# gfxdisp/FovVideoVDP

Hardware: AMD Instinct MI355X
Metric: Mpixels/s (test+ref) at 4Kx60f; JOD delta vs reference (higher is better)
Workload: dtype f32

## Files before the change

fovvideovdp_amd/csrc/aux_kernels.hpp:

```cpp
#pragma once
struct FinalizeArgs {
    const float* partial;
    float* Q;
    int n_bands, n, q_stride, q_col0, tc;
    float inv_beta;
    int nblk[FVVDP_MAX_BANDS];
    long long off[FVVDP_MAX_BANDS];
    float npx[FVVDP_MAX_BANDS];
};

__device__ __forceinline__ void finalize_one(const FinalizeArgs& a, const int b, const int cc, const int s, const int lane) {
    float q = 0.0f;
    if (cc < a.tc) {
        const float* p = a.partial + a.off[b] + (size_t)s * a.nblk[b] * 2 + cc;
        double sum = 0.0;
        for (int k = lane; k < a.nblk[b]; k += 64) sum += (double)p[2 * k];
#pragma unroll
        for (int off = 32; off > 0; off >>= 1) sum += __shfl_down(sum, off, 64);
        q = (float)pow(sum / (double)a.npx[b], (double)a.inv_beta);
    }
    if (lane == 0) a.Q[((size_t)b * 2 + cc) * a.q_stride + a.q_col0 + s] = q;
}

__global__ __launch_bounds__(64) void finalize_kernel(const FinalizeArgs a) {
    const int i = blockIdx.x;
    finalize_one(a, i / (2 * a.n), (i / a.n) % 2, i % a.n, (int)threadIdx.x);
}

struct PoolArgs {
    const float* Q;
    int n_bands, n_ch, n_frames, q_stride;
    float beta_sch, beta_tch, beta_t, w_transient, jod_a, beta_jod;
    float* out;
};

__device__ __forceinline__ float pool_pow(float x, float p) { return p == 1.0f ? x : powf(x, p); }

__device__ __forceinline__ float pool_frame(const PoolArgs& a, const int f) {
    float qt = 0.0f;
    for (int c = 0; c < a.n_ch; ++c) {
        const float wc = (a.n_ch == 2 && c == 1) ? a.w_transient : 1.0f;
        float qs = 0.0f;
        for (int b = 0; b < a.n_bands; ++b)
            qs += pool_pow(fabsf(a.Q[((size_t)b * 2 + c) * a.q_stride + f] * wc), a.beta_sch);
        qs = pool_pow(qs, 1.0f / a.beta_sch);
        qt += pool_pow(qs, a.beta_tch);
    }
    qt = pool_pow(qt, 1.0f / a.beta_tch);
    return pool_pow(qt, a.beta_t);
}

__device__ __forceinline__ void pool_jod_body(const PoolArgs& a, double* s_part, const int tid) {
    double acc = 0.0;
    if (tid < 256) {
        for (int f = tid; f < a.n_frames; f += 256) acc += (double)pool_frame(a, f);
        s_part[tid] = acc;
    }
    __syncthreads();
    for (int o = 128; o >= 1; o >>= 1) {
        if (tid < o) s_part[tid] += s_part[tid + o];
        __syncthreads();
    }
    if (tid == 0) {
        const float q_all = pool_pow((float)(s_part[0] / (double)a.n_frames), 1.0f / a.beta_t);
        const float sgn = a.jod_a < 0.0f ? -1.0f : 1.0f;
        a.out[0] = sgn * powf(powf(fabsf(a.jod_a), 1.0f / a.beta_jod) * q_all, a.beta_jod) + 10.0f;
    }
}

__global__ __launch_bounds__(256) void pool_jod_kernel(const PoolArgs a) {
    __shared__ double s_part[256];
    pool_jod_body(a, s_part, (int)threadIdx.x);
}

struct PoolColsArgs {
    PoolArgs p;
    int n_cols;
};
// ... 209 lines not shown
```

fovvideovdp_amd/csrc/fvvdp_hip.hip:

```cpp
#include <hip/hip_runtime.h>
#include <hip/hip_fp16.h>

#include <algorithm>
#include <cmath>
#include <cfloat>
#include <cstdarg>
#include <cstdio>
#include <cstdlib>
#include <cstring>
#include <vector>

#include "fvvdp_hip.h"
#include "fvvdp_hip_images.h"
#include "fvvdp_hip_gaze.h"

static thread_local char g_err[512] = "";

static int fail(int code, const char* fmt, ...) {
    va_list ap;
    va_start(ap, fmt);
    vsnprintf(g_err, sizeof(g_err), fmt, ap);
    va_end(ap);
    return code;
}
// ... 37 lines not shown
};
static CtxEnv read_env() {
    CtxEnv e;
    auto num = [](const char* name, int dflt) { const char* v = getenv(name); return (v && v[0]) ? atoi(v) : dflt; };
    if (const char* v = getenv("FVVDP_ALLOC")) e.alloc_malloc = strcmp(v, "malloc") == 0;
    e.vmm_chunk = (size_t)(num("FVVDP_VMM_CHUNK_MB", 0) > 0 ? num("FVVDP_VMM_CHUNK_MB", 0) : 0) << 20;
    e.probe_n = num("FVVDP_PLACEMENT_PROBE", -1);
    e.probe_extra = num("FVVDP_PLACEMENT_EXTRA", -1);
    if (const char* v = getenv("FVVDP_PLACEMENT_MIXED_TBS")) e.probe_mixed = (float)atof(v);
    if (const char* v = getenv("FVVDP_BAND_INRANGE")) e.inrange_off = v[0] == '0';
    if (const char* v = getenv("FVVDP_BAND_FUSE")) e.fuse_mode = (v[0] == '0' || v[0] == '1') ? v[0] - '0' : -1;
    e.band2_kr = num("FVVDP_BAND2_KR", 0);
    e.band2_kr2 = num("FVVDP_BAND2_KR2", -1);
    e.band2_wpb = num("FVVDP_BAND2_WPB", 0);
    if (const char* v = getenv("FVVDP_K1_TICKET")) e.k1_ticket = v[0] != '0' ? 1 : 0;
    if (const char* v = getenv("FVVDP_BAND2_TICKET")) e.band2_ticket = v[0] != '0' ? 1 : 0;
    if (const char* v = getenv("FVVDP_LEVEL0_SPLIT")) e.level0_split = v[0] != '0' ? 1 : 0;
    e.temporal_scalar = getenv("FVVDP_TEMPORAL_SCALAR") != nullptr;
    e.debug_variant = getenv("FVVDP_DEBUG_VARIANT") != nullptr;
    e.yuv_general = getenv("FVVDP_YUV_GENERAL_MATRIX") != nullptr;
    e.gaze_group = num("FVVDP_GAZE_GROUP", 0);
    return e;
}

struct VmmBlock {
    void* ptr;
    size_t size;
    std::vector<hipMemGenericAllocationHandle_t> handles;
};
struct fvvdp_ctx {
    CtxEnv env;
    int W = 0, H = 0, n_bands = 0, P = 0, max_frames = 0;
    fvvdp_params prm{};
    double rho_band[FVVDP_MAX_BANDS + 1]{};
    int lw[FVVDP_MAX_BANDS + 1]{}, lh[FVVDP_MAX_BANDS + 1]{};
    float* level[FVVDP_MAX_BANDS + 1]{};
    float* level0_hi = nullptr;
    int sel_phase = 9;
    int sel_n = 0;
    int sel_kept = -1;
    float sel_us[8] = {0, 0, 0, 0, 0, 0, 0, 0};
    int level0_kind = 0;
    int level0_kind_hi = -1;
    long long n_sync = 0, n_alloc = 0, n_free = 0;
    bool created = false;
    bool lum_known = false;
    int lum_state = 0;
    int lum_hold = 0;
    int lum_top = 0;
    float lum_lo = 0.0f, lum_hi = 0.0f, lum_width = 0.0f;
    float* partial = nullptr;
    long long partial_off[FVVDP_MAX_BANDS]{};
    int max_blk[FVVDP_MAX_BANDS]{};
    int* d_ticket = nullptr;
    size_t partial_floats = 0;
    float4* csf = nullptr;
    float4* csf_y = nullptr;
    bool csf_set = false;
    float y_first = 0, y_inv_step = 0, y_lo = 0, y_hi = 0;
    std::vector<float> h_lut3[2];
    float h_axes[3][FVVDP_LUT_N]{};
    float* d_axes = nullptr;
    float4* sublut[FVVDP_MAX_BANDS]{};
    float4* rmap[FVVDP_MAX_BANDS]{};
    int sub_rw[FVVDP_MAX_BANDS]{}, sub_ilo[FVVDP_MAX_BANDS]{};
    fvvdp_geom sub_geom{};
    const float* map_vx[FVVDP_MAX_BANDS]{};
    const float* map_vy[FVVDP_MAX_BANDS]{};
    const float* map_rm[FVVDP_MAX_BANDS]{};
    float map_rm_max[FVVDP_MAX_BANDS]{}, map_rm_min[FVVDP_MAX_BANDS]{};
    bool maps_set = false;
    bool sub_valid = false;
    float rho_lo = 0, rho_hi = 0, ecc_lo = 0, ecc_hi = 0;
    bool lut3_set[2] = {false, false};
    float* d_fix = nullptr;
    float* d_taps = nullptr;
    int* d_idx = nullptr;
    float* lum_buf = nullptr;
    size_t lum_floats = 0;
    float* heat[FVVDP_MAX_BANDS + 1]{};
    unsigned int* colour_ws = nullptr;
    size_t scratch = 0;
    std::vector<VmmBlock> vmm;
    long long wave_capacity = 4096;
    long long wave_capacity2 = 4096;
    bool timing = false;
    std::vector<std::pair<hipEvent_t, hipEvent_t>> ev[FVVDP_MAX_BANDS + 2];
    float t_ms[FVVDP_MAX_BANDS + 2]{};
    int t_cnt[FVVDP_MAX_BANDS + 2]{};
};

static const size_t VMM_MIN_BYTES = (size_t)16 << 20;
static const size_t VMM_BIG_BYTES = (size_t)256 << 20;

static int vmm_alloc(fvvdp_ctx* c, void** out, size_t bytes);
static void vmm_free_all(fvvdp_ctx* c);

template <typename T>
static int dev_alloc(fvvdp_ctx* c, T** p, size_t count) {
    void* q = nullptr;
    const size_t bytes = count * sizeof(T);
    if (!c->env.alloc_malloc && bytes >= VMM_MIN_BYTES && vmm_alloc(c, &q, bytes) == FVVDP_OK) {
    } else {
        q = nullptr;
        (void)hipGetLastError();
        hipError_t e = hipMalloc(&q, bytes);
        if (e != hipSuccess) return fail(FVVDP_ENOMEM, "hipMalloc(%zu bytes) failed: %s", bytes, hipGetErrorString(e));
// ... 147 lines not shown

static void choose_level0(fvvdp_ctx* c);

extern "C" int fvvdp_ctx_create(fvvdp_ctx** out, int width, int height, int n_bands, int planes, int max_frames,
                                const double* h_rho_band, const fvvdp_params* prm) {
    if (!out || !prm || !h_rho_band) return fail(FVVDP_EINVAL, "null argument");
    if (planes != 2 && planes != 4) return fail(FVVDP_EINVAL, "planes must be 2 (image) or 4 (video), got %d", planes);
    if (n_bands < 1 || n_bands > FVVDP_MAX_BANDS) return fail(FVVDP_EINVAL, "n_bands %d out of range", n_bands);
    if (max_frames < 1) return fail(FVVDP_EINVAL, "max_frames must be >= 1");
    if (width < 4 || height < 4) return fail(FVVDP_EINVAL, "frame %dx%d too small", width, height);
    fvvdp_ctx* c = new fvvdp_ctx();
    c->env = read_env();
    c->W = width;
    c->H = height;
    c->n_bands = n_bands;
    c->P = planes;
    c->max_frames = max_frames;
    c->prm = *prm;
    int w = width, h = height;
    for (int i = 0; i <= n_bands; ++i) {
        c->lw[i] = w;
        c->lh[i] = h;
        c->rho_band[i] = h_rho_band[i];
        if (i < n_bands && (w < 2 || h < 2)) {
            delete c;
            return fail(FVVDP_EINVAL, "pyramid level %d is %dx%d: too many bands for this frame size", i, w, h);
        }
        w = (w + 1) / 2;
        h = (h + 1) / 2;
    }
    int rc = FVVDP_OK;
    for (int i = 0; i <= n_bands && rc == FVVDP_OK; ++i) {
        rc = dev_alloc(c, &c->level[i], (size_t)max_frames * c->lw[i] * c->lh[i] * planes);
    }
    size_t off = 0;
    for (int b = 0; b < n_bands; ++b) {
        const int n_strips = band_strips(c->lw[b + 1]);
        const int max_chunks = (c->lh[b + 1] + 1) / 2;
        c->max_blk[b] = n_strips * max_chunks;
    }
    for (int b = 0; b + 1 < n_bands; ++b) {
        const int blk2 = band2_strips(c->lw[b + 1]) * c->lh[b + 2];
        if (blk2 > c->max_blk[b]) c->max_blk[b] = blk2;
        if (blk2 > c->max_blk[b + 1]) c->max_blk[b + 1] = blk2;
    }
    for (int b = 0; b < n_bands; ++b) {
        c->partial_off[b] = (long long)off;
        off += (size_t)max_frames * c->max_blk[b] * 2;
    }
    c->partial_floats = off;
    if (rc == FVVDP_OK) rc = dev_alloc(c, &c->partial, off);
    if (rc == FVVDP_OK) {
        float* q = nullptr;
        rc = dev_alloc(c, &q, 16);
        c->d_ticket = reinterpret_cast<int*>(q);
    }
    if (rc == FVVDP_OK) rc = dev_alloc(c, &c->csf, (size_t)n_bands * FVVDP_LUT_N);
    if (rc == FVVDP_OK) rc = dev_alloc(c, &c->csf_y, (size_t)FVVDP_LUT_N);
    if (rc == FVVDP_OK) rc = dev_alloc(c, &c->d_fix, (size_t)max_frames * 2);
    if (rc == FVVDP_OK) rc = dev_alloc(c, &c->d_taps, (size_t)2 * FVVDP_MAX_TAPS);
    if (rc == FVVDP_OK) rc = dev_alloc(c, &c->d_idx, (size_t)max_frames + FVVDP_MAX_TAPS);
    if (rc != FVVDP_OK) {
        fvvdp_ctx_destroy(c);
        return rc;
    }
    {
        int dev = 0, cus = 256, per_cu = 16;
        if (hipGetDevice(&dev) == hipSuccess) {
            hipDeviceProp_t prop;
            if (hipGetDeviceProperties(&prop, dev) == hipSuccess) cus = prop.multiProcessorCount;
        }
        hipError_t e = (planes == 4)
            ? hipOccupancyMaxActiveBlocksPerMultiprocessor(&per_cu, band_kernel<4, false, 0>, 64, 0)
            : hipOccupancyMaxActiveBlocksPerMultiprocessor(&per_cu, band_kernel<2, false, 0>, 64, 0);
        if (e != hipSuccess || per_cu < 1) per_cu = 16;
        c->wave_capacity = (long long)per_cu * cus;
        int per_cu2 = 16;
        e = (planes == 4) ? hipOccupancyMaxActiveBlocksPerMultiprocessor(&per_cu2, band2_kernel<4, false>, 64, 0)
                          : hipOccupancyMaxActiveBlocksPerMultiprocessor(&per_cu2, band2_kernel<2, false>, 64, 0);
        if (e != hipSuccess || per_cu2 < 1) per_cu2 = 16;
        c->wave_capacity2 = (long long)per_cu2 * cus;
    }
    choose_level0(c);
    if (!c->level[0]) {
        fvvdp_ctx_destroy(c);
        return fail(FVVDP_ENOMEM, "no device memory for pyramid level 0");
    }
    c->created = true;
    *out = c;
    return FVVDP_OK;
}

extern "C" void fvvdp_ctx_destroy(fvvdp_ctx* c) {
    if (!c) return;
    (void)hipDeviceSynchronize();
    for (int i = 0; i <= FVVDP_MAX_BANDS; ++i)
        dev_free(c, c->level[i]);
    dev_free(c, c->level0_hi);
    dev_free(c, c->partial);
    dev_free(c, c->d_ticket);
    if (c->csf) (void)hipFree(c->csf);
    if (c->csf_y) (void)hipFree(c->csf_y);
    for (int i = 0; i <= FVVDP_MAX_BANDS; ++i)
        dev_free(c, c->heat[i]);
    if (c->colour_ws) (void)hipFree(c->colour_ws);
    if (c->d_fix) (void)hipFree(c->d_fix);
    if (c->d_taps) (void)hipFree(c->d_taps);
    if (c->d_idx) (void)hipFree(c->d_idx);
// ... 167 lines not shown
    return lo >= c->prm.lbkg_min &&
           c->prm.contrast_max * lo > c->lum_width &&
           lo >= 2.0f * c->y_lo && hi <= 0.5f * c->y_hi;
}

static int temporal_channels_core(fvvdp_ctx* c, const void* d_test, const void* d_ref, int dtype, int C,
                                  size_t chan_stride, size_t frame_stride, const fvvdp_eotf* eotf,
                                  const float* h_rgb2y, const int32_t* h_frame_idx, const int32_t* h_frame_idx1,
                                  const float* h_taps, int fl, int n_out, int slot0, int32_t* d_oob_flag, void* stream) {
    if (!c || !d_test || !d_ref || !eotf || !h_frame_idx || !h_taps) return fail(FVVDP_EINVAL, "null argument");
    if (dtype < FVVDP_U8 || dtype > FVVDP_F32) return fail(FVVDP_EINVAL, "Only uint8, uint16 and float32 is currently supported");
    if (C != 1 && C != 3) return fail(FVVDP_EINVAL, "The content must have either 1 or 3 colour channels.");
    if (C == 3 && !h_rgb2y) return fail(FVVDP_EINVAL, "rgb2y weights required for C == 3");
    if (fl < 1 || fl > FVVDP_MAX_TAPS) return fail(FVVDP_EINVAL, "filter length %d out of range", fl);
    if (c->P == 2 && fl != 1) return fail(FVVDP_EINVAL, "still-image context (planes == 2) needs fl == 1");
    if (n_out < 1 || slot0 < 0 || slot0 + n_out > c->max_frames) return fail(FVVDP_EINVAL, "slots [%d,%d) exceed max_frames %d", slot0, slot0 + n_out, c->max_frames);
    if (eotf->kind == FVVDP_EOTF_LUT && (dtype == FVVDP_F32 || !eotf->d_lut)) return fail(FVVDP_EINVAL, "FVVDP_EOTF_LUT needs an integer source and a table");
    if (eotf->kind != FVVDP_EOTF_LUT && dtype == FVVDP_U8) return fail(FVVDP_EINVAL, "uint8 sources need FVVDP_EOTF_LUT (uint16: table or closed form)");
    hipStream_t st = reinterpret_cast<hipStream_t>(stream);
    const int HW = c->W * c->H;
    luminance_slots(c, slot0, n_out);
    luminance_range(c, eotf, C, h_rgb2y, h_taps, fl);
    Timed tm(c, 0, st);
    const bool ring64 = (c->P == 4) && fl > 32 && fl <= 64 && !c->env.temporal_scalar &&
                        k1_ring64_ok(dtype, C, eotf->kind);
    const bool ring_ok = ((c->P == 4) && (fl <= 32)) || ring64;
    if (ring_ok) {
        const int FL = fl <= 8 ? 8 : (fl <= 16 ? 16 : (fl <= 32 ? 32 : 64));
        const int max_out = T_MAX_IDX - (FL - 1);
        auto run = [&](int t_begin, int t_end) -> int {
            for (int t0 = t_begin; t0 < t_end; t0 += max_out) {
                const int nn = (t_end - t0) < max_out ? (t_end - t0) : max_out;
                TemporalArgs a;
                memset(&a, 0, sizeof(a));
                a.src[0] = d_test;
                a.src[1] = d_ref;
                a.chan_stride = chan_stride;
                a.frame_stride = frame_stride;
                a.C = C;
                a.HW = HW;
                a.e = make_eotf(eotf);
                if (C == 3) { a.w[0] = h_rgb2y[0]; a.w[1] = h_rgb2y[1]; a.w[2] = h_rgb2y[2]; } else { a.w[0] = 1.0f; }
                a.n_out = nn;
                a.fl = fl;
                a.out = level_addr(c, 0, slot0 + t0);
                a.oob = d_oob_flag;
                for (int k = 0; k < fl; ++k) { a.taps2[k][0] = h_taps[k]; a.taps2[k][1] = h_taps[fl + k]; }
                const int pad = FL - fl;
                for (int u = 0; u < FL - 1 + nn; ++u) {
                    const int src = t0 + u - pad;
                    a.idx[u] = h_frame_idx[src < 0 ? 0 : src];
                    a.idx1[u] = h_frame_idx1 ? h_frame_idx1[src < 0 ? 0 : src] : a.idx[u];
                }
                const int PXv = k1_px(FL);
                const int es = dtype == FVVDP_U8 ? 1 : (dtype == FVVDP_U16 ? 2 : 4);
                const bool vec_ok = !c->env.temporal_scalar && (HW % PXv == 0) && (HW >= PXv) &&
                                    (chan_stride % PXv == 0) && (frame_stride % PXv == 0) &&
                                    (reinterpret_cast<uintptr_t>(d_test) % (size_t)(es * PXv) == 0) &&
                                    (reinterpret_cast<uintptr_t>(d_ref) % (size_t)(es * PXv) == 0);
                if (vec_ok) {
                    const bool tickets = FL == 16 && c->env.k1_ticket != 0;
                    if (tickets && dtype == FVVDP_U8 && c->d_ticket) {
                        if (hipMemsetAsync(c->d_ticket, 0, sizeof(int), st) == hipSuccess) a.ticket = c->d_ticket;
                        else (void)hipGetLastError();
                    }
                    k1_launch_vec(FL, dtype, a, st);
                } else if (FL == 64) {
                    return fail(FVVDP_EINVAL, "source pointers must be aligned to their element size");
                } else {
                    k1_launch_ring(FL, dtype, a, st);
                }
            }
            return FVVDP_OK;
        };
        {
            const int rc = run(0, n_out);
            if (rc != FVVDP_OK) return rc;
        }
    } else if (c->P == 4 && fl > 32 && fl <= 64 && !h_frame_idx1 && !c->env.temporal_scalar &&
               fl - 1 + n_out <= T_MAX_IDX && k1_ring64_ok(FVVDP_F32, 1, FVVDP_EOTF_NONE)) {
        const int total = fl - 1 + n_out;
        std::vector<int> uniq(h_frame_idx, h_frame_idx + total);
        std::sort(uniq.begin(), uniq.end());
        uniq.erase(std::unique(uniq.begin(), uniq.end()), uniq.end());
        const int nu = (int)uniq.size();
        {
            const int rc = grow_lum_buf(c, (size_t)2 * nu * HW, fl, st);
            if (rc != FVVDP_OK) return rc;
        }
        LumArgs la;
        memset(&la, 0, sizeof(la));
        la.src[0] = d_test;
        la.src[1] = d_ref;
        la.chan_stride = chan_stride;
        la.frame_stride = frame_stride;
        la.C = C;
        la.HW = HW;
        la.e = make_eotf(eotf);
        if (C == 3) { la.w[0] = h_rgb2y[0]; la.w[1] = h_rgb2y[1]; la.w[2] = h_rgb2y[2]; } else { la.w[0] = 1.0f; }
        la.n_frames = nu;
        la.out = c->lum_buf;
        la.oob = d_oob_flag;
        for (int k = 0; k < nu; ++k) la.fr[k] = uniq[k];
        k1_launch_luminance(dtype, la, st);
        std::vector<int32_t> pos(total);
        for (int u = 0; u < total; ++u) pos[u] = (int32_t)(std::lower_bound(uniq.begin(), uniq.end(), h_frame_idx[u]) - uniq.begin());
        fvvdp_eotf none;
        memset(&none, 0, sizeof(none));
        none.kind = FVVDP_EOTF_NONE;
        HIP_TRY(hipGetLastError());
        const bool timing = c->timing;
        c->timing = false;
        c->lum_hold += 1;
        const int rc2 = temporal_channels_core(c, c->lum_buf, c->lum_buf + (size_t)nu * HW, FVVDP_F32, 1, 0, (size_t)HW, &none, nullptr,
                                               pos.data(), nullptr, h_taps, fl, n_out, slot0, d_oob_flag, stream);
        c->timing = timing;
        c->lum_hold -= 1;
        return rc2;
    } else {
        if (h_frame_idx1) return fail(FVVDP_EINVAL, "per-frame source pointers are supported for video with fl <= 32 (uint8: 64) only");
        if (fl - 1 + n_out > c->max_frames + FVVDP_MAX_TAPS) return fail(FVVDP_EINVAL, "too many frames for one call");
        GenericArgs a;
        memset(&a, 0, sizeof(a));
        if (fl <= 32 && fl - 1 + n_out <= T_MAX_IDX) {
            a.inline_tables = 1;
            for (int k = 0; k < 2 * fl; ++k) a.taps_i[k] = h_taps[k];
            for (int k = 0; k < fl - 1 + n_out; ++k) a.idx_i[k] = h_frame_idx[k];
        } else {
            HIP_TRY(hipStreamSynchronize(st));
            c->n_sync += 1;
            HIP_TRY(hipMemcpy(c->d_taps, h_taps, sizeof(float) * 2 * fl, hipMemcpyHostToDevice));
            HIP_TRY(hipMemcpy(c->d_idx, h_frame_idx, sizeof(int) * (fl - 1 + n_out), hipMemcpyHostToDevice));
        }
        a.src[0] = d_test;
        a.src[1] = d_ref;
        a.chan_stride = chan_stride;
        a.frame_stride = frame_stride;
        a.C = C;
        a.HW = HW;
        a.e = make_eotf(eotf);
        if (C == 3) { a.w[0] = h_rgb2y[0]; a.w[1] = h_rgb2y[1]; a.w[2] = h_rgb2y[2]; } else { a.w[0] = 1.0f; }
        a.n_out = n_out;
        a.fl = fl;
        a.out = level_addr(c, 0, slot0);
        a.oob = d_oob_flag;
        a.taps = c->d_taps;
        a.idx = c->d_idx;
        k1_launch_generic(c->P, dtype, a, st);
    }
    HIP_TRY(hipGetLastError());
    return FVVDP_OK;
}

extern "C" int fvvdp_temporal_channels(fvvdp_ctx* c, const void* d_test, const void* d_ref, int dtype, int C,
                                       size_t chan_stride, size_t frame_stride, const fvvdp_eotf* eotf,
                                       const float* h_rgb2y, const int32_t* h_frame_idx, const float* h_taps, int fl,
                                       int n_out, int slot0, int32_t* d_oob_flag, void* stream) {
    return temporal_channels_core(c, d_test, d_ref, dtype, C, chan_stride, frame_stride, eotf, h_rgb2y, h_frame_idx, nullptr,
                                  h_taps, fl, n_out, slot0, d_oob_flag, stream);
}

extern "C" int fvvdp_temporal_channels_frames(fvvdp_ctx* c, const void* const* h_test_frames, const void* const* h_ref_frames,
                                              int n_frames, int dtype, int C, size_t chan_stride, const fvvdp_eotf* eotf,
                                              const float* h_rgb2y, const int32_t* h_frame_idx, const float* h_taps, int fl,
                                              int n_out, int slot0, int32_t* d_oob_flag, void* stream) {
    if (!c || !h_test_frames || !h_ref_frames || !h_frame_idx) return fail(FVVDP_EINVAL, "null argument");
    if (n_frames < 1 || n_frames > 65536) return fail(FVVDP_EINVAL, "n_frames out of range");
    if (dtype < FVVDP_U8 || dtype > FVVDP_F32) return fail(FVVDP_EINVAL, "Only uint8, uint16 and float32 is currently supported");
    if (fl < 1 || fl > ((eotf && k1_ring64_ok(dtype, C, eotf->kind)) ? 64 : 32) || c->P != 4)
        return fail(FVVDP_EUNSUPPORTED, "per-frame source pointers: video contexts with fl <= 32 (uint8, float luminance: 64) only");
    const size_t es = dtype == FVVDP_U8 ? 1 : (dtype == FVVDP_U16 ? 2 : 4);
    const void* const* fr[2] = {h_test_frames, h_ref_frames};
    uintptr_t base[2];
    size_t gran = 4;
    for (int s = 0; s < 2; ++s) {
        base[s] = UINTPTR_MAX;
        for (int i = 0; i < n_frames; ++i) {
            if (!fr[s][i]) return fail(FVVDP_EINVAL, "null frame pointer");
            const uintptr_t p = reinterpret_cast<uintptr_t>(fr[s][i]);
            if (p % es) return fail(FVVDP_EINVAL, "frame pointer not aligned to its element size");
            if (p < base[s]) base[s] = p;
        }
        for (int i = 0; i < n_frames; ++i)
            if ((reinterpret_cast<uintptr_t>(fr[s][i]) - base[s]) % (es * 4)) gran = 1;
    }
    std::vector<int32_t> off[2];
    for (int s = 0; s < 2; ++s) {
        off[s].resize(n_frames);
        for (int i = 0; i < n_frames; ++i) {
            const uintptr_t d = (reinterpret_cast<uintptr_t>(fr[s][i]) - base[s]) / (es * gran);
            if (d > 0x7FFFFFFFu) return fail(FVVDP_EUNSUPPORTED, "frames are too far apart in memory for 31-bit frame indices");
            off[s][i] = (int32_t)d;
        }
    }
    const int total = fl - 1 + n_out;
    std::vector<int32_t> i0(total), i1(total);
    for (int u = 0; u < total; ++u) {
        const int f = h_frame_idx[u];
        if (f < 0 || f >= n_frames) return fail(FVVDP_EINVAL, "frame index %d out of range", f);
        i0[u] = off[0][f];
        i1[u] = off[1][f];
    }
    return temporal_channels_core(c, reinterpret_cast<const void*>(base[0]), reinterpret_cast<const void*>(base[1]), dtype, C,
// ... 408 lines not shown
            a.mrm = c->map_rm[b];
        }
        a.rho_band = (float)c->rho_band[b];
        a.rho_lo = c->rho_lo;
        a.rho_hi = c->rho_hi;
        a.ecc_lo = c->ecc_lo;
        a.ecc_hi = c->ecc_hi;
        for (int ax = 0; ax < 3; ++ax) {
            a.first[ax] = c->h_axes[ax][0];
            a.inv_step[ax] = (float)(FVVDP_LUT_N - 1) / (c->h_axes[ax][FVVDP_LUT_N - 1] - c->h_axes[ax][0]);
            const double step = ((double)c->h_axes[ax][FVVDP_LUT_N - 1] - (double)c->h_axes[ax][0]) / (FVVDP_LUT_N - 1);
            a.frac_scale[ax] = (float)(step / (step + 1e-6));
            a.grid_off[ax] = -a.first[ax] * a.inv_step[ax];
        }
        a.frame_w = c->W;
        a.frame_h = c->H;
        a.rmap = geom ? c->rmap[b] : nullptr;
        a.rmap_w = (c->lw[b] + 1) / 2;
    }
    {
        const size_t lut_b = (size_t)FOV_PLANE * c->sub_rw[b] * sizeof(float4);
        const size_t lds_static = sizeof(float4) * FVVDP_LUT_N + sizeof(float2) * 3 * FVVDP_LUT_N;
        a.lut_lds = (fov && lut_b <= 56 * 1024 && lut_b + (size_t)c->lh[b] * sizeof(float) + lds_static <= 64 * 1024) ? 1 : 0;
    }
}

static int bands_forward_core(fvvdp_ctx* c, int slot0, int n, float* d_Q, int q_stride, int q_col0, const float* h_fixation,
                              const fvvdp_geom* geom, const fvvdp_band_maps* maps, const fvvdp_pool_params* pool,
                              float* d_jod, void* stream, int plan_n = 0) {
    if (plan_n < 1) plan_n = n;
    if (!c || !d_Q) return fail(FVVDP_EINVAL, "null argument");
    if (slot0 < 0 || n < 1 || slot0 + n > c->max_frames) return fail(FVVDP_EINVAL, "slots [%d,%d) exceed max_frames %d", slot0, slot0 + n, c->max_frames);
    if (pool) {
        if (!d_jod) return fail(FVVDP_EINVAL, "null argument");
        int rc = check_pool_params(pool);
        if (rc != FVVDP_OK) return rc;
    }
    const bool last_batch = (q_col0 + n == q_stride);
    const bool pool_now = pool && last_batch;
    if (n < 1 || n > c->max_frames) return fail(FVVDP_EINVAL, "n=%d exceeds max_frames=%d", n, c->max_frames);
    if (q_col0 < 0 || q_col0 + n > q_stride) return fail(FVVDP_EINVAL, "Q columns out of range");
    const bool fov = h_fixation != nullptr;
    if (fov && !geom && !c->maps_set) return fail(FVVDP_EINVAL, "foveated mode needs the display geometry (or fvvdp_ctx_set_view_maps)");
    if (fov && !(c->lut3_set[0] && (c->P == 2 || c->lut3_set[1]))) return fail(FVVDP_ESTATE, "fvvdp_ctx_set_csf_3d not called");
    if (!fov && !c->csf_set) return fail(FVVDP_ESTATE, "fvvdp_ctx_set_csf_1d not called");
    hipStream_t st = reinterpret_cast<hipStream_t>(stream);
    if (fov) {
        HIP_TRY(hipMemcpyAsync(c->d_fix, h_fixation, sizeof(float) * 2 * n, hipMemcpyHostToDevice, st));
        int rc = build_sublut(c, geom, st);
        if (rc != FVVDP_OK) return rc;
    }
    FinalizeArgs fa;
    memset(&fa, 0, sizeof(fa));
    bool any_maps = false;
    if (maps)
        for (int b = 0; b < c->n_bands; ++b) any_maps = any_maps || maps[b].d_D || maps[b].d_contrast || maps[b].d_lbkg || maps[b].d_S;
    const int fuse_mode = c->env.fuse_mode;
    const bool fuse_ok = !fov && !any_maps && fuse_mode != 0;
    for (int b = 0; b < c->n_bands; ++b) {
        const bool big = (long long)c->lw[b] * c->lh[b] >= 500000;
        if (fuse_ok && (big || fuse_mode == 1) && b + 1 < c->n_bands && c->lw[b + 1] >= 4 && c->lh[b + 1] >= 4 &&
            c->lw[b + 2] >= 2 && c->lh[b + 2] >= 2) {
            Band2Args a;
            memset(&a, 0, sizeof(a));
            a.A = level_addr(c, b, b == 0 ? slot0 : 0);
            a.Gc = c->level[b + 2];
            a.w = c->lw[b];
            a.h = c->lh[b];
            a.wb = c->lw[b + 1];
            a.hb = c->lh[b + 1];
            a.wc = c->lw[b + 2];
            a.hc = c->lh[b + 2];
            a.n_strips = band2_strips(a.wb);
            chunking2(a.hc, a.n_strips, plan_n, c->wave_capacity2, c->env.band2_kr, a.n_chunks, a.kr);
            a.n_big = a.n_chunks;
            a.kr2 = a.kr;
            a.n_frames = n;
            {
                const long long waves = (long long)plan_n * a.n_strips * a.n_chunks;
                int kr2 = (waves >= 2 * c->wave_capacity2 && a.n_chunks >= 3 && a.kr >= 16) ? (a.kr + 3) / 4 : 0;
                if (c->env.band2_kr2 >= 0) kr2 = c->env.band2_kr2;
                if (kr2 >= 1 && kr2 < a.kr && a.n_chunks >= 2) {
                    a.n_big = a.n_chunks - 1;
                    a.kr2 = kr2;
                    a.n_chunks = a.n_big + (a.hc - a.n_big * a.kr + kr2 - 1) / kr2;
                }
            }
            a.mulA = (b == 0) ? 1.0f : 2.0f;
            a.mulB = 2.0f;
            a.csfA = c->csf + (size_t)b * FVVDP_LUT_N;
            a.csfB = c->csf + (size_t)(b + 1) * FVVDP_LUT_N;
            a.y_first = c->y_first;
            a.y_inv_step = c->y_inv_step;
            a.ly_lo = log2f(c->y_lo);
            a.ly_hi = log2f(c->y_hi);
            a.lg_gain = log2f(c->prm.sens_gain);
            a.lg_k = log2f(c->prm.mask_k);
            a.p = c->prm.mask_p;
            a.q0 = c->prm.mask_q[0];
            a.q1 = c->prm.mask_q[1];
            a.beta = c->prm.beta;
            a.lbkg_min = c->prm.lbkg_min;
            a.cmax = c->prm.contrast_max;
            a.lg_dmax = log2f(c->prm.d_max);
            a.partialA = c->partial + c->partial_off[b];
            a.partialB = c->partial + c->partial_off[b + 1];
            const int nblk = a.n_strips * a.n_chunks;
            if (nblk > c->max_blk[b] || nblk > c->max_blk[b + 1]) return fail(FVVDP_ESTATE, "internal: partial buffer too small");
            {
                Timed tm(c, 1 + b, st);
                const bool inrange = clamps_never_bind(c, b, 2);
                int wpb = (a.w >= 2560 && a.n_strips % BAND2_WPB_MAX == 0) ? BAND2_WPB_MAX : 1;
                { const int v = c->env.band2_wpb; if (v >= 1 && v <= BAND2_WPB_MAX && a.n_strips % v == 0) wpb = v; }
                const int n_items = (a.n_strips / wpb) * a.n_chunks * n;
                const long long waves2 = (long long)n * a.n_strips * a.n_chunks;
                bool tickets = c->d_ticket && (c->env.band2_ticket == 1 ||
                                               (c->env.band2_ticket != 0 && waves2 >= 2 * c->wave_capacity2 && wpb == BAND2_WPB_MAX && a.w >= 2560));
                if (tickets && hipMemsetAsync(c->d_ticket, 0, 16 * sizeof(int), st) != hipSuccess) { (void)hipGetLastError(); tickets = false; }
                a.n_items = n_items;
                a.tickets = tickets ? c->d_ticket : nullptr;
                const int n_wg = tickets ? ((n_items + n_items / 8 + 7) / 8 * 8) : n_items;
                const dim3 grid2((unsigned int)n_wg), block2(64 * wpb);
                if (c->env.debug_variant)
                    fprintf(stderr, "fvvdp: levels %d+%d: band2_kernel<%d, %s>, luminance range %s [%g, %g], widest plane range %g, %d waves per workgroup"
                                    ", n_strips %d, kr %d, kr2 %d, n_big %d, n_chunks %d, tickets %s\n",
                                 b, b + 1, c->P, inrange ? "true" : "false", c->lum_state == 1 ? "known" : "unknown", c->lum_lo, c->lum_hi, c->lum_width, wpb,
                                 a.n_strips, a.kr, a.kr2, a.n_big, a.n_chunks, tickets ? "on" : "off");
                if (c->P == 4) {
                    if (inrange) hipLaunchKernelGGL((band2_kernel<4, true>), grid2, block2, 0, st, a);
                    else hipLaunchKernelGGL((band2_kernel<4, false>), grid2, block2, 0, st, a);
                } else {
                    if (inrange) hipLaunchKernelGGL((band2_kernel<2, true>), grid2, block2, 0, st, a);
                    else hipLaunchKernelGGL((band2_kernel<2, false>), grid2, block2, 0, st, a);
                }
            }
            for (int bb = b; bb <= b + 1; ++bb) {
                fa.nblk[bb] = nblk;
                fa.off[bb] = c->partial_off[bb];
                fa.npx[bb] = (float)c->lw[bb] * (float)c->lh[bb];
            }
            ++b;
            continue;
        }
        BandArgs a;
        fill_band_args(c, b, slot0, plan_n, fov, geom, a);
        a.partial = c->partial + c->partial_off[b];
        bool dbg = false;
        if (maps) {
            a.dD = maps[b].d_D;
            a.dC = maps[b].d_contrast;
            a.dL = maps[b].d_lbkg;
            a.dS = maps[b].d_S;
            dbg = a.dD || a.dC || a.dL || a.dS;
        }
        const int nblk = a.n_strips * a.n_chunks;
        if (nblk > c->max_blk[b]) return fail(FVVDP_ESTATE, "internal: partial buffer too small");
        a.n_items = nblk * n;
        {
            Timed tm(c, 1 + b, st);
            if (c->P == 4) launch_band<4>(a, nblk * n, dbg, fov, st);
            else launch_band<2>(a, nblk * n, dbg, fov, st);
        }
        fa.nblk[b] = nblk;
        fa.off[b] = c->partial_off[b];
        fa.npx[b] = (float)a.w * (float)a.h;
    }
    fa.partial = c->partial;
    fa.Q = d_Q;
    fa.n_bands = c->n_bands;
    fa.n = n;
    fa.q_stride = q_stride;
    fa.q_col0 = q_col0;
    fa.tc = c->P / 2;
    fa.inv_beta = 1.0f / c->prm.beta;
    {
        Timed tm(c, 1 + c->n_bands, st);
        const int total = c->n_bands * 2 * n;
        hipLaunchKernelGGL(finalize_kernel, dim3(total), dim3(64), 0, st, fa);
    }
    if (pool_now) {
        PoolArgs pa;
        fill_pool_args(pa, d_Q, c->n_bands, 2, q_stride, q_stride, pool, d_jod);
        hipLaunchKernelGGL(pool_jod_kernel, dim3(1), dim3(256), 0, st, pa);
    }
    HIP_TRY(hipGetLastError());
    return FVVDP_OK;
}

extern "C" int fvvdp_bands_forward(fvvdp_ctx* c, int n, float* d_Q, int q_stride, int q_col0, const float* h_fixation,
                                   const fvvdp_geom* geom, const fvvdp_band_maps* maps, void* stream) {
    return bands_forward_core(c, 0, n, d_Q, q_stride, q_col0, h_fixation, geom, maps, nullptr, nullptr, stream);
}

extern "C" int fvvdp_bands_forward_pool(fvvdp_ctx* c, int n, float* d_Q, int q_stride, int q_col0, const float* h_fixation,
                                        const fvvdp_geom* geom, const fvvdp_band_maps* maps, const fvvdp_pool_params* pool,
                                        float* d_jod, void* stream) {
    if (!pool) return fail(FVVDP_EINVAL, "null argument");
    return bands_forward_core(c, 0, n, d_Q, q_stride, q_col0, h_fixation, geom, maps, pool, d_jod, stream);
}

static size_t gaze_row_floats(int width, int height, int n_bands, int n, size_t* off) {
    size_t fl = 0;
    int w = width, h = height;
    for (int b = 0; b < n_bands; ++b) {
        const int wc = (w + 1) / 2, hc = (h + 1) / 2;
        if (off) off[b] = fl;
        fl += (size_t)n * band_strips(wc) * ((hc + 1) / 2) * 2;
        w = wc;
        h = hc;
    }
    return (fl + 63) / 64 * 64;
}

extern "C" int fvvdp_gaze_workspace(int width, int height, int n_bands, int n_gazes, int n, size_t* bytes) {
    if (!bytes) return fail(FVVDP_EINVAL, "null argument");
    if (width < 1 || height < 1 || n_gazes < 1 || n < 1 || n_bands < 1 || n_bands > FVVDP_MAX_BANDS)
        return fail(FVVDP_EINVAL, "bad shape: %dx%d, %d bands, %d gazes, %d frames", width, height, n_bands, n_gazes, n);
    *bytes = (size_t)n_gazes * gaze_row_floats(width, height, n_bands, n, nullptr) * sizeof(float);
    return FVVDP_OK;
}

template <int P>
static void launch_multigaze(const MultiGazeArgs& m, int ng, hipStream_t st) {
    const dim3 grid((m.b.n_items + FOV_WPB - 1) / FOV_WPB), block(64 * FOV_WPB);
    const size_t lds = (size_t)FOV_PLANE * m.b.rw * sizeof(float4) + (size_t)m.b.h * sizeof(float);
    if (ng == 8) hipLaunchKernelGGL((multigaze_kernel<P, 8>), grid, block, lds, st, m);
    else if (ng == 4) hipLaunchKernelGGL((multigaze_kernel<P, 4>), grid, block, lds, st, m);
    else if (ng == 2) hipLaunchKernelGGL((multigaze_kernel<P, 2>), grid, block, lds, st, m);
    else hipLaunchKernelGGL((multigaze_kernel<P, 1>), grid, block, lds, st, m);
}

static int bands_forward_gazes_core(fvvdp_ctx* c, int n, int n_gazes, const float* d_gaze, size_t gaze_stride, float* d_Q,
                                    int q_stride, int q_col0, const fvvdp_geom* geom, void* d_work, size_t work_bytes,
                                    const fvvdp_pool_params* pool, float* d_jod, void* stream) {
    if (!c || !d_gaze || !d_Q || !geom || !d_work) return fail(FVVDP_EINVAL, "null argument");
    if (pool) {
        if (!d_jod) return fail(FVVDP_EINVAL, "null argument");
        int rc = check_pool_params(pool);
// ... 513 lines not shown
```

fovvideovdp_amd/csrc/temporal_kernels.hpp:

```cpp
#pragma once
enum { SRC_U8 = 0, SRC_U16 = 1, SRC_F32 = 2 };

struct EotfDev {
    int kind;
    float scale;
    float y_black;
    float y_peak;
    float gamma;
    float l_min, l_max;
    const float* lut;
};

struct OobMax {
    float m = 0.0f;
};
__device__ __forceinline__ void note_oob(bool& b, float V) { b = b || (V > 1.0f) || (V < 0.0f); }
__device__ __forceinline__ void note_oob(OobMax& b, float V) {
    const float over = V - 1.0f;
    asm("v_max3_f32 %0, %0, %1, -%2" : "+v"(b.m) : "v"(over), "v"(V));
}
__device__ __forceinline__ bool is_oob(bool b) { return b; }
__device__ __forceinline__ bool is_oob(const OobMax& b) { return b.m > 0.0f; }

template <int KIND, typename B>
// ... 101 lines not shown
            }
            const float wc = (c == 0) ? w0 : ((c == 1) ? w1 : w2);
            if (e.kind != FVVDP_EOTF_LUT) {
#pragma unroll
                for (int i = 0; i < PX; ++i) o[i] = __fmul_rn(eotf_f32((float)code[i] * (1.0f / 65535.0f), e, bad), wc);
            } else {
#pragma unroll
                for (int i = 0; i < PX; ++i) o[i] = __fmul_rn(lut_entry(lut16, code[i], e), wc);
            }
        } else {
            const float* q = reinterpret_cast<const float*>(p) + off;
            float V[PX];
            if constexpr (PX == 4) {
                const float4 t = *reinterpret_cast<const float4*>(q);
                V[0] = t.x; V[1] = t.y; V[2] = t.z; V[3] = t.w;
            } else if constexpr (PX == 2) {
                const float2 t = *reinterpret_cast<const float2*>(q);
                V[0] = t.x; V[1] = t.y;
            } else {
                V[0] = *q;
            }
            const float wc = (c == 0) ? w0 : ((c == 1) ? w1 : w2);
#pragma unroll
            for (int i = 0; i < PX; ++i) o[i] = __fmul_rn(eotf_f32(V[i], e, bad), wc);
        }
    }

    __device__ __forceinline__ void lum(size_t foff, float (&L)[PX], bool& bad) const {
        if (C == 3) {
            float a[PX], b[PX], c[PX];
            chan(base, foff, a, 0, bad);
            chan(base, foff + chan_stride, b, 1, bad);
            chan(base, foff + 2 * chan_stride, c, 2, bad);
#pragma unroll
            for (int i = 0; i < PX; ++i) L[i] = __fadd_rn(__fadd_rn(a[i], b[i]), c[i]);
        } else {
            chan(base, foff, L, 0, bad);
        }
    }
};

#define T_MAX_IDX 320
struct TemporalArgs {
    const void* src[2];
    size_t chan_stride, frame_stride;
    int C, HW;
    EotfDev e;
    float w[3];
    int n_out;
    int fl;
    L0Addr out;
    int* oob;
    int* ticket;
    float taps2[64][2];
    int idx[T_MAX_IDX];
    int idx1[T_MAX_IDX];
};

__device__ __forceinline__ float lut_entry(const float* lut, unsigned code, const EotfDev& e) {
    return fminf(fmaxf(lut[code], e.l_min), e.l_max);
}

__device__ __forceinline__ void build_lutw(float* lutw, const EotfDev& e, int C, const float* w, int tid, int nthreads) {
    for (int i = tid; i < 256; i += nthreads) {
        const float l = lut_entry(e.lut, i, e);
        if (C == 3) {
            lutw[i] = __fmul_rn(l, w[0]);
            lutw[256 + i] = __fmul_rn(l, w[1]);
            lutw[512 + i] = __fmul_rn(l, w[2]);
        } else {
            lutw[i] = l;
        }
    }
}

template <int SRC, int PX>
struct RawPx {
    unsigned int wd[PX];
    __device__ __forceinline__ unsigned int code(int i) const { return wd[i]; }
    __device__ __forceinline__ float value(int i) const { return __uint_as_float(wd[i]); }
};

template <int SRC, int PX>
__device__ __forceinline__ RawPx<SRC, PX> load_raw(const void* base, size_t off, const int (&px)[PX]) {
    RawPx<SRC, PX> r;
#pragma unroll
    for (int i = 0; i < PX; ++i) {
        if constexpr (SRC == SRC_U8) r.wd[i] = reinterpret_cast<const unsigned char*>(base)[off + px[i]];
        else if constexpr (SRC == SRC_U16) r.wd[i] = reinterpret_cast<const unsigned short*>(base)[off + px[i]];
        else r.wd[i] = reinterpret_cast<const unsigned int*>(base)[off + px[i]];
    }
    return r;
}

template <int SRC, int PX>
struct RawFrame {
    RawPx<SRC, PX> ch[3];
};

template <int SRC, int PX>
__device__ __forceinline__ RawFrame<SRC, PX> fetch_frame(const void* base, size_t off, size_t chan_stride, int C,
                                                         const int (&px)[PX]) {
    RawFrame<SRC, PX> f;
    f.ch[0] = load_raw<SRC, PX>(base, off, px);
    if (C == 3) {
        f.ch[1] = load_raw<SRC, PX>(base, off + chan_stride, px);
// ... 289 lines not shown
        f.ch[2] = load_vec<SRC, PX>(base, off + 2 * chan_stride);
    } else {
        f.ch[1] = f.ch[0];
        f.ch[2] = f.ch[0];
    }
    return f;
}

__device__ __forceinline__ void wave_lds_order() {
    __builtin_amdgcn_fence(__ATOMIC_RELEASE, "wavefront");
    __builtin_amdgcn_wave_barrier();
    __builtin_amdgcn_fence(__ATOMIC_ACQUIRE, "wavefront");
}

constexpr int K1_STORE_AUX = 2;
template <int FL, int PX, int SRC, int TD, int CC, int KIND>
__device__ __forceinline__ void temporal_vec_body(const TemporalArgs& a, const float* lutw, float4* s_t, const int block = (int)blockIdx.x) {
    typedef const int __attribute__((address_space(4)))* karg_int_p;
    typedef const char __attribute__((address_space(4)))* karg_p;
    const karg_p ka = (karg_p)__builtin_amdgcn_kernarg_segment_ptr();
    const karg_int_p idx0 = (karg_int_p)(ka + offsetof(TemporalArgs, idx));
    const karg_int_p idx1 = (karg_int_p)(ka + offsetof(TemporalArgs, idx1));
    const int lane = threadIdx.x & 63;
    const int p0 = block * (64 * PX);
    const int pl = min(p0 + lane * PX, a.HW - PX);
    const float w[3] = {CC == 3 ? a.w[0] : 1.0f, a.w[1], a.w[2]};
    OobMax bad;
    v2f ring[FL][PX];
    const int total = FL - 1 + a.n_out;
    static_assert(FL % TD == 0, "prefetch slots are indexed with the unrolled ring position");
    RawVecFrame<SRC, PX> nx[TD][2];
    auto prefetch = [&](int v, RawVecFrame<SRC, PX>& f0, RawVecFrame<SRC, PX>& f1) {
        const int vv = min(v, total - 1);
        f0 = fetch_vec<SRC, PX>(a.src[0], (size_t)idx0[vv] * a.frame_stride + pl, a.chan_stride, CC);
        f1 = fetch_vec<SRC, PX>(a.src[1], (size_t)idx1[vv] * a.frame_stride + pl, a.chan_stride, CC);
    };
    constexpr bool PAIRS = (SRC == SRC_F32 || SRC == SRC_U16) && KIND >= 0 && KIND != FVVDP_EOTF_LUT;
    auto push = [&](const RawVecFrame<SRC, PX>& c0, const RawVecFrame<SRC, PX>& c1, v2f (&slot)[PX]) {
        if constexpr (PAIRS) {
            frame_lum_pairs<SRC, PX, CC, KIND>(c0, c1, w, a.e, slot, bad);
#pragma unroll
            for (int i = 0; i < PX; ++i) asm volatile("" : "+v"(slot[i]));
        } else {
            float L0[PX], L1[PX];
            frame_lum<SRC, PX, RawVecFrame<SRC, PX>, KIND>(c0, CC, lutw, a.e.lut, w, a.e, L0, bad);
            frame_lum<SRC, PX, RawVecFrame<SRC, PX>, KIND>(c1, CC, lutw, a.e.lut, w, a.e, L1, bad);
#pragma unroll
            for (int i = 0; i < PX; ++i) {
                slot[i] = v2f{L0[i], L1[i]};
                asm volatile("" : "+v"(slot[i]));
            }
        }
    };
    constexpr int HB_REGS = FL == 64 ? 16 : ((FL == 32 && RawVec<SRC, PX>::WORDS > 1) ? 24 : 48);
    constexpr int HB = (HB_REGS / (6 * RawVec<SRC, PX>::WORDS)) > 0 ? (HB_REGS / (6 * RawVec<SRC, PX>::WORDS)) : 1;
#pragma unroll
    for (int u0 = 0; u0 < FL - 1; u0 += HB) {
        RawVecFrame<SRC, PX> h[HB][2];
#pragma unroll
        for (int d = 0; d < HB; ++d)
            if (u0 + d < FL - 1) prefetch(u0 + d, h[d][0], h[d][1]);
        if (u0 + HB >= FL - 1) {
#pragma unroll
            for (int d = 0; d < TD; ++d) prefetch(FL - 1 + d, nx[(FL - 1 + d) % TD][0], nx[(FL - 1 + d) % TD][1]);
        }
#pragma unroll
        for (int d = 0; d < HB; ++d)
            if (u0 + d < FL - 1) push(h[d][0], h[d][1], ring[u0 + d]);
        __builtin_amdgcn_sched_barrier(0);
    }
    unsigned int soff[PX];
#pragma unroll
    for (int i = 0; i < PX; ++i) soff[i] = (p0 + i * 64 + lane < a.HW) ? (unsigned int)(p0 + i * 64 + lane) * 16u : FVVDP_NO_STORE;
    const unsigned int frame_bytes = (unsigned int)a.HW * 16u;
    __builtin_amdgcn_s_waitcnt(0x0F70);
    for (int t0 = 0; t0 < a.n_out; t0 += FL) {
#pragma unroll
        for (int j = 0; j < FL; ++j) {
            const int t = t0 + j;
            if (t >= a.n_out) break;
            const int u = (FL - 1 + j) % FL;
            if constexpr (RawVec<SRC, PX>::WORDS == 1) {
                const RawVecFrame<SRC, PX> cur0 = nx[u % TD][0], cur1 = nx[u % TD][1];
                prefetch(FL - 1 + t + TD, nx[u % TD][0], nx[u % TD][1]);
                push(cur0, cur1, ring[u]);
            } else {
                push(nx[u % TD][0], nx[u % TD][1], ring[u]);
                __builtin_amdgcn_sched_barrier(0);
                prefetch(FL - 1 + t + TD, nx[u % TD][0], nx[u % TD][1]);
            }
            __builtin_amdgcn_sched_barrier(0);
            v2f accS[PX], accT[PX];
            bool first_tap = true;
            karg_p tp = ka + offsetof(TemporalArgs, taps2);
            if constexpr (FL > 16) asm volatile("" : "+s"(tp));
#pragma unroll
            for (int c = FL / TAPC - 1; c >= 0; --c) {
                const vtapf tc = *(karg_taps_p)(tp + c * (8 * TAPC));
#pragma unroll
                for (int kk = TAPC - 1; kk >= 0; --kk) {
                    const int k = c * TAPC + kk;
                    const int sl = (u - k + 2 * FL) % FL;
                    const v2f f = v2f{tc[2 * kk], tc[2 * kk + 1]};
#pragma unroll
                    for (int i = 0; i < PX; ++i) {
                        if (first_tap) fir_tap_first(accS[i], accT[i], ring[sl][i], f);
                        else fir_tap(accS[i], accT[i], ring[sl][i], f);
                    }
                    first_tap = false;
                }
            }
            wave_lds_order();
#pragma unroll
            for (int i = 0; i < PX; ++i)
                s_t[lane * (PX + 1) + i] = make_float4(accS[i].x, accS[i].y, accT[i].x, accT[i].y);
            wave_lds_order();
            int t_opaque = t;
            asm volatile("" : "+s"(t_opaque));
            const __amdgpu_buffer_rsrc_t o = level_rsrc(l0_frame(a.out, t_opaque), frame_bytes);
#pragma unroll
            for (int i = 0; i < PX; ++i) {
// ... 11 lines not shown
__device__ __forceinline__ void temporal_vec_cc(const TemporalArgs& a, const float* lutw, float4* s_t, const int block = (int)blockIdx.x) {
    if (a.C == 3) temporal_vec_body<FL, PX, SRC, TD, 3, KIND>(a, lutw, s_t, block);
    else temporal_vec_body<FL, PX, SRC, TD, 1, KIND>(a, lutw, s_t, block);
}

constexpr int K1_WAVES8 = 4;
constexpr int K1_WAVES16 = 4;
constexpr int K1_WAVES32 = 3;
constexpr int K1_WAVES64 = 3;
constexpr int K1_WAVESX8 = 3;
constexpr int K1_WAVESF8 = 3;
constexpr int K1_WAVESX16 = 4;
constexpr int K1_WAVESX32 = 2;
constexpr int k1_waves(int FL, int SRC) {
    return SRC == SRC_U8 ? (FL == 8 ? K1_WAVES8 : (FL == 16 ? K1_WAVES16 : (FL == 32 ? K1_WAVES32 : K1_WAVES64)))
                         : FL == 64 ? K1_WAVES64 : (FL == 8 ? (SRC == SRC_F32 ? K1_WAVESF8 : K1_WAVESX8) : (FL == 16 ? K1_WAVESX16 : K1_WAVESX32));
}
constexpr int K1_WPB8 = 4;
constexpr int k1_wpb(int FL) { return FL == 8 ? K1_WPB8 : 1; }
template <int FL, int PX, int SRC, int TD = 1>
__global__ __launch_bounds__(64 * k1_wpb(FL), k1_waves(FL, SRC))
void temporal_vec_kernel(const TemporalArgs a_byval) {

    const TemporalArgs& a = *(const TemporalArgs*)__builtin_amdgcn_kernarg_segment_ptr();
    (void)a_byval;
    static_assert(TD == 1, "one frame of raw samples in flight (temporal_launch.hpp)");
    constexpr int WPB = k1_wpb(FL);
    __shared__ float lutw[SRC == SRC_U8 ? 768 : 1];
    __shared__ float4 s_t_all[WPB][64 * (PX + 1)];
    if constexpr (SRC == SRC_U8) build_lutw(lutw, a.e, a.C, a.w, threadIdx.x, 64 * WPB);
    __syncthreads();
    const int wave = WPB > 1 ? __builtin_amdgcn_readfirstlane((int)(threadIdx.x >> 6)) : 0;
    float4* const s_t = s_t_all[wave];
    const int block0 = (int)blockIdx.x * WPB + wave;
    if constexpr (WPB > 1) {
        if (block0 * (64 * PX) >= a.HW) return;
    }
    if constexpr (SRC == SRC_U8 && FL == 16) {
        typedef const char __attribute__((address_space(4)))* karg_p;
        int block = block0;
        const int n_blocks = (a.HW + 64 * PX - 1) / (64 * PX);
        for (;;) {
            int next = 0x7fffffff;
            {
                karg_p ka = (karg_p)__builtin_amdgcn_kernarg_segment_ptr();
                asm volatile("" : "+s"(ka));
                int* const tk = *(int* const __attribute__((address_space(4)))*)(ka + offsetof(TemporalArgs, ticket));
                if (tk && threadIdx.x == 0) next = (int)gridDim.x + atomicAdd(tk, 1);
            }
            temporal_vec_cc<FL, PX, SRC, TD, FVVDP_EOTF_LUT>(a, lutw, s_t, block);
            block = __builtin_amdgcn_readfirstlane(next);
            if (block >= n_blocks) break;
            wave_lds_order();
        }
    } else if constexpr (SRC == SRC_U8) {
        temporal_vec_cc<FL, PX, SRC, TD, FVVDP_EOTF_LUT>(a, lutw, s_t, block0);
    } else if constexpr (FL == 64) {
        if (a.C == 3 && a.e.kind == FVVDP_EOTF_SRGB) temporal_vec_body<FL, PX, SRC, TD, 3, FVVDP_EOTF_SRGB>(a, lutw, s_t, block0);
        else if (a.C == 3 && a.e.kind == FVVDP_EOTF_PQ) temporal_vec_body<FL, PX, SRC, TD, 3, FVVDP_EOTF_PQ>(a, lutw, s_t, block0);
        else if constexpr (SRC == SRC_F32) {
            if (a.C == 1 && a.e.kind == FVVDP_EOTF_NONE) temporal_vec_body<FL, PX, SRC, TD, 1, FVVDP_EOTF_NONE>(a, lutw, s_t, block0);
        }
    } else {
        switch (a.e.kind) {
            case FVVDP_EOTF_SRGB: temporal_vec_cc<FL, PX, SRC, TD, FVVDP_EOTF_SRGB>(a, lutw, s_t, block0); break;
            case FVVDP_EOTF_GAMMA: temporal_vec_cc<FL, PX, SRC, TD, FVVDP_EOTF_GAMMA>(a, lutw, s_t, block0); break;
            case FVVDP_EOTF_PQ: temporal_vec_cc<FL, PX, SRC, TD, FVVDP_EOTF_PQ>(a, lutw, s_t, block0); break;
            case FVVDP_EOTF_LINEAR: temporal_vec_cc<FL, PX, SRC, TD, FVVDP_EOTF_LINEAR>(a, lutw, s_t, block0); break;
            case FVVDP_EOTF_ABSOLUTE: temporal_vec_cc<FL, PX, SRC, TD, FVVDP_EOTF_ABSOLUTE>(a, lutw, s_t, block0); break;
            case FVVDP_EOTF_LUT:
                if constexpr (SRC == SRC_U16) temporal_vec_cc<FL, PX, SRC, TD, FVVDP_EOTF_LUT>(a, lutw, s_t, block0);
                break;
            default: temporal_vec_cc<FL, PX, SRC, TD, FVVDP_EOTF_NONE>(a, lutw, s_t, block0); break;
        }
    }
}

struct YuvArgs {
    const void* src[2];
    size_t frame_stride;
    int W, H, uvw, uvh;
    int chroma420;
    float wy, wc;
    float m[9];
    EotfDev e;
    float w[3];
    int n_out, fl;
    L0Addr out;
    int* oob;
    float taps2[32][2];
    int idx[T_MAX_IDX];
};

template <typename T, typename B>
__device__ __forceinline__ float yuv_lum(const T* __restrict__ f, const YuvArgs& a, int p, B& bad) {
    const int HW = a.W * a.H;
    const int y = p / a.W, x = p - y * a.W;
    const float Yf = fminf(fmaxf(a.wy * (float)f[p] - (16.0f / 219.0f), 0.0f), 1.0f);
    const T* U = f + HW;
    const T* V = U + a.uvw * a.uvh;
    auto cf = [&](const T* pl, int yy, int xx) {
        return fminf(fmaxf(a.wc * (float)pl[yy * a.uvw + xx] - (128.0f / 224.0f), -0.5f), 0.5f);
    };
    float u, v;
    if (a.chroma420) {
        const float sy = fmaxf(((float)y + 0.5f) * 0.5f - 0.5f, 0.0f), sx = fmaxf(((float)x + 0.5f) * 0.5f - 0.5f, 0.0f);
// ... 553 lines not shown
```

Baseline: 231,000.

## Self-reset ticket counters in kernels and skip reloading repeated warmup frames

Removes the hipMemsetAsync calls issued before each ticketed launch. The kernels now reset their own counters: the last K1 workgroup zeroes its ticket, and the finalize kernel zeroes the band2 ticket sets. Each band2 launch gets its own ticket slot, so one band no longer has to wait on a memset before the next. It also adds a bitmask of temporal-filter warmup frames that repeat the previous index, so those frames are copied from the ring register instead of loaded again. The cost is more complex state tracking, including dirty flags used as a fallback when a reset fails.

Result: faster. 234,100, median of 6 (+1.4%).

```diff
diff --git a/fovvideovdp_amd/csrc/aux_kernels.hpp b/fovvideovdp_amd/csrc/aux_kernels.hpp
--- a/fovvideovdp_amd/csrc/aux_kernels.hpp
+++ b/fovvideovdp_amd/csrc/aux_kernels.hpp
@@ -7,6 +7,8 @@
     int nblk[FVVDP_MAX_BANDS];
     long long off[FVVDP_MAX_BANDS];
     float npx[FVVDP_MAX_BANDS];
+    int* reset;
+    int n_reset;
 };
 
 __device__ __forceinline__ void finalize_one(const FinalizeArgs& a, const int b, const int cc, const int s, const int lane) {
@@ -24,6 +26,8 @@
 
 __global__ __launch_bounds__(64) void finalize_kernel(const FinalizeArgs a) {
     const int i = blockIdx.x;
+    if (i == 0 && threadIdx.x == 0 && a.reset)
+        for (int k = 0; k < a.n_reset; ++k) __hip_atomic_store(a.reset + k, 0, __ATOMIC_RELAXED, __HIP_MEMORY_SCOPE_AGENT);
     finalize_one(a, i / (2 * a.n), (i / a.n) % 2, i % a.n, (int)threadIdx.x);
 }
 
diff --git a/fovvideovdp_amd/csrc/fvvdp_hip.hip b/fovvideovdp_amd/csrc/fvvdp_hip.hip
--- a/fovvideovdp_amd/csrc/fvvdp_hip.hip
+++ b/fovvideovdp_amd/csrc/fvvdp_hip.hip
@@ -113,7 +113,11 @@
     float* partial = nullptr;
     long long partial_off[FVVDP_MAX_BANDS]{};
     int max_blk[FVVDP_MAX_BANDS]{};
+    static constexpr int TICKET_SETS = FVVDP_MAX_BANDS / 2;
+    static constexpr int K1_TICKET_AT = 16 * TICKET_SETS;
+    static constexpr int TICKET_INTS = K1_TICKET_AT + 16;
     int* d_ticket = nullptr;
+    bool band2_tickets_dirty = false, k1_ticket_dirty = false;
     size_t partial_floats = 0;
     float4* csf = nullptr;
     float4* csf_y = nullptr;
@@ -367,8 +371,13 @@
     if (rc == FVVDP_OK) rc = dev_alloc(c, &c->partial, off);
     if (rc == FVVDP_OK) {
         float* q = nullptr;
-        rc = dev_alloc(c, &q, 16);
+        rc = dev_alloc(c, &q, fvvdp_ctx::TICKET_INTS);
         c->d_ticket = reinterpret_cast<int*>(q);
+        if (rc == FVVDP_OK && hipMemset(c->d_ticket, 0, fvvdp_ctx::TICKET_INTS * sizeof(int)) != hipSuccess) {
+            (void)hipGetLastError();
+            dev_free(c, c->d_ticket);
+            c->d_ticket = nullptr;
+        }
     }
     if (rc == FVVDP_OK) rc = dev_alloc(c, &c->csf, (size_t)n_bands * FVVDP_LUT_N);
     if (rc == FVVDP_OK) rc = dev_alloc(c, &c->csf_y, (size_t)FVVDP_LUT_N);
@@ -642,6 +651,8 @@
                     a.idx[u] = h_frame_idx[src < 0 ? 0 : src];
                     a.idx1[u] = h_frame_idx1 ? h_frame_idx1[src < 0 ? 0 : src] : a.idx[u];
                 }
+                for (int u = 1; u < FL - 1; ++u)
+                    if (a.idx[u] == a.idx[u - 1] && a.idx1[u] == a.idx1[u - 1]) a.rep |= 1ull << u;
                 const int PXv = k1_px(FL);
                 const int es = dtype == FVVDP_U8 ? 1 : (dtype == FVVDP_U16 ? 2 : 4);
                 const bool vec_ok = !c->env.temporal_scalar && (HW % PXv == 0) && (HW >= PXv) &&
@@ -651,8 +662,9 @@
                 if (vec_ok) {
                     const bool tickets = FL == 16 && c->env.k1_ticket != 0;
                     if (tickets && dtype == FVVDP_U8 && c->d_ticket) {
-                        if (hipMemsetAsync(c->d_ticket, 0, sizeof(int), st) == hipSuccess) a.ticket = c->d_ticket;
-                        else (void)hipGetLastError();
+                        int* const tk = c->d_ticket + fvvdp_ctx::K1_TICKET_AT;
+                        if (c->k1_ticket_dirty && hipMemsetAsync(tk, 0, 2 * sizeof(int), st) != hipSuccess) (void)hipGetLastError();
+                        else { a.ticket = tk; c->k1_ticket_dirty = true; }
                     }
                     k1_launch_vec(FL, dtype, a, st);
                 } else if (FL == 64) {
@@ -739,6 +751,7 @@
         k1_launch_generic(c->P, dtype, a, st);
     }
     HIP_TRY(hipGetLastError());
+    c->k1_ticket_dirty = false;
     return FVVDP_OK;
 }
 
@@ -1253,6 +1266,12 @@
     }
     FinalizeArgs fa;
     memset(&fa, 0, sizeof(fa));
+    int ticket_sets = 0;
+    if (c->band2_tickets_dirty && c->d_ticket) {
+        if (hipMemsetAsync(c->d_ticket, 0, 16 * fvvdp_ctx::TICKET_SETS * sizeof(int), st) == hipSuccess) c->band2_tickets_dirty = false;
+        else (void)hipGetLastError();
+    }
+    const bool counters_ok = c->d_ticket && !c->band2_tickets_dirty;
     bool any_maps = false;
     if (maps)
         for (int b = 0; b < c->n_bands; ++b) any_maps = any_maps || maps[b].d_D || maps[b].d_contrast || maps[b].d_lbkg || maps[b].d_S;
@@ -1315,11 +1334,12 @@
                 { const int v = c->env.band2_wpb; if (v >= 1 && v <= BAND2_WPB_MAX && a.n_strips % v == 0) wpb = v; }
                 const int n_items = (a.n_strips / wpb) * a.n_chunks * n;
                 const long long waves2 = (long long)n * a.n_strips * a.n_chunks;
-                bool tickets = c->d_ticket && (c->env.band2_ticket == 1 ||
-                                               (c->env.band2_ticket != 0 && waves2 >= 2 * c->wave_capacity2 && wpb == BAND2_WPB_MAX && a.w >= 2560));
-                if (tickets && hipMemsetAsync(c->d_ticket, 0, 16 * sizeof(int), st) != hipSuccess) { (void)hipGetLastError(); tickets = false; }
+                const bool tickets = counters_ok && ticket_sets < fvvdp_ctx::TICKET_SETS &&
+                                     (c->env.band2_ticket == 1 ||
+                                      (c->env.band2_ticket != 0 && waves2 >= 2 * c->wave_capacity2 && wpb == BAND2_WPB_MAX && a.w >= 2560));
                 a.n_items = n_items;
-                a.tickets = tickets ? c->d_ticket : nullptr;
+                a.tickets = tickets ? c->d_ticket + 16 * ticket_sets++ : nullptr;
+                if (tickets) c->band2_tickets_dirty = true;
                 const int n_wg = tickets ? ((n_items + n_items / 8 + 7) / 8 * 8) : n_items;
                 const dim3 grid2((unsigned int)n_wg), block2(64 * wpb);
                 if (c->env.debug_variant)
@@ -1377,6 +1397,8 @@
     {
         Timed tm(c, 1 + c->n_bands, st);
         const int total = c->n_bands * 2 * n;
+        fa.reset = ticket_sets ? c->d_ticket : nullptr;
+        fa.n_reset = 16 * ticket_sets;
         hipLaunchKernelGGL(finalize_kernel, dim3(total), dim3(64), 0, st, fa);
     }
     if (pool_now) {
@@ -1385,6 +1407,7 @@
         hipLaunchKernelGGL(pool_jod_kernel, dim3(1), dim3(256), 0, st, pa);
     }
     HIP_TRY(hipGetLastError());
+    c->band2_tickets_dirty = false;
     return FVVDP_OK;
 }
 
diff --git a/fovvideovdp_amd/csrc/temporal_kernels.hpp b/fovvideovdp_amd/csrc/temporal_kernels.hpp
--- a/fovvideovdp_amd/csrc/temporal_kernels.hpp
+++ b/fovvideovdp_amd/csrc/temporal_kernels.hpp
@@ -177,6 +177,7 @@
     L0Addr out;
     int* oob;
     int* ticket;
+    unsigned long long rep;
     float taps2[64][2];
     int idx[T_MAX_IDX];
     int idx1[T_MAX_IDX];
@@ -572,6 +573,8 @@
             }
         }
     };
+    const unsigned long long rep = a.rep;
+    auto repeated = [&](int u) { return ((rep >> u) & 1ull) != 0ull; };
     constexpr int HB_REGS = FL == 64 ? 16 : ((FL == 32 && RawVec<SRC, PX>::WORDS > 1) ? 24 : 48);
     constexpr int HB = (HB_REGS / (6 * RawVec<SRC, PX>::WORDS)) > 0 ? (HB_REGS / (6 * RawVec<SRC, PX>::WORDS)) : 1;
 #pragma unroll
@@ -579,14 +582,21 @@
         RawVecFrame<SRC, PX> h[HB][2];
 #pragma unroll
         for (int d = 0; d < HB; ++d)
-            if (u0 + d < FL - 1) prefetch(u0 + d, h[d][0], h[d][1]);
+            if (u0 + d < FL - 1 && !repeated(u0 + d)) prefetch(u0 + d, h[d][0], h[d][1]);
         if (u0 + HB >= FL - 1) {
 #pragma unroll
             for (int d = 0; d < TD; ++d) prefetch(FL - 1 + d, nx[(FL - 1 + d) % TD][0], nx[(FL - 1 + d) % TD][1]);
         }
 #pragma unroll
         for (int d = 0; d < HB; ++d)
-            if (u0 + d < FL - 1) push(h[d][0], h[d][1], ring[u0 + d]);
+            if (u0 + d < FL - 1) {
+                if (u0 + d > 0 && repeated(u0 + d)) {
+#pragma unroll
+                    for (int i = 0; i < PX; ++i) ring[u0 + d][i] = ring[u0 + d - 1][i];
+                } else {
+                    push(h[d][0], h[d][1], ring[u0 + d]);
+                }
+            }
         __builtin_amdgcn_sched_barrier(0);
     }
     unsigned int soff[PX];
@@ -704,6 +714,16 @@
             block = __builtin_amdgcn_readfirstlane(next);
             if (block >= n_blocks) break;
             wave_lds_order();
+        }
+        {
+            karg_p ka = (karg_p)__builtin_amdgcn_kernarg_segment_ptr();
+            asm volatile("" : "+s"(ka));
+            int* const tk = *(int* const __attribute__((address_space(4)))*)(ka + offsetof(TemporalArgs, ticket));
+            if (tk && threadIdx.x == 0 &&
+                __hip_atomic_fetch_add(tk + 1, 1, __ATOMIC_ACQ_REL, __HIP_MEMORY_SCOPE_AGENT) == (int)gridDim.x - 1) {
+                __hip_atomic_store(tk, 0, __ATOMIC_RELAXED, __HIP_MEMORY_SCOPE_AGENT);
+                __hip_atomic_store(tk + 1, 0, __ATOMIC_RELAXED, __HIP_MEMORY_SCOPE_AGENT);
+            }
         }
     } else if constexpr (SRC == SRC_U8) {
         temporal_vec_cc<FL, PX, SRC, TD, FVVDP_EOTF_LUT>(a, lutw, s_t, block0);
```
